# wavey-ai/soundkit

Measured on AMD Instinct MI355X. Metric: AAC-LC 1024-sample frames/s (whole node) + xrealtime, batch=4096 48 kHz stereo, higher is better.
Workload: dtype f32 (synthesis f32; s16 between the kernels as in the reference; FIR: the 16-bit samples as 2 x f16 exactly, the f32 taps as 2 x f16 to 2^-24, f32 accumulate; 1.0e-7 rel. RMS vs f64)

## Files before the change

soundkit_amd/csrc/fir_bf16.hip:

```cpp
#include "sk_device.h"

#include <cstdlib>
#include <type_traits>

namespace sk {

namespace {

typedef float f32x4 __attribute__((ext_vector_type(4)));
typedef __bf16 bf16x8 __attribute__((ext_vector_type(8)));
typedef uint32_t u32x4 __attribute__((ext_vector_type(4)));
typedef uint32_t u32x2 __attribute__((ext_vector_type(2)));

constexpr int kRing = 192;
constexpr int kPlaneBytes = 2 * kRing;
__host__ __device__ constexpr int row_bytes(int planes) { return planes * kPlaneBytes + 32; }
constexpr int kWindows = 10;
__device__ constexpr int kProducts[kWindows] = {1, 3, 6, 6, 6, 6, 6, 3, 3, 1};
__host__ __device__ constexpr int products_of(int s, bool in16) { return in16 && kProducts[s] > 5 ? 5 : kProducts[s]; }
__device__ constexpr int kProductsF16[kWindows] = {kFirProductsF16[0], kFirProductsF16[1], kFirProductsF16[2], kFirProductsF16[3], kFirProductsF16[4],
                                                     kFirProductsF16[5], kFirProductsF16[6], kFirProductsF16[7], kFirProductsF16[8], kFirProductsF16[9]};
__host__ __device__ constexpr int products_of(int s, bool in16, bool f16) { return f16 ? kProductsF16[s] : products_of(s, in16); }
#ifndef SK_BF_AHEAD
#define SK_BF_AHEAD 3
#endif
constexpr int kAhead = SK_BF_AHEAD;

__host__ __device__ constexpr int ring_index(int rho) { return ((rho % kRing) + kRing) % kRing; }

template <bool PACKED>
__device__ __forceinline__ size_t row_base_offset(const FirArgs &a, uint32_t row) {
    if (!PACKED) return (size_t)row * a.in_stride;
    const uint32_t sh = a.in_ch - 1;
    return (size_t)(row >> sh) * a.in_group_stride + (size_t)((row & sh) << 10);
}

template <bool PACKED>
__device__ __forceinline__ size_t time_offset(const FirArgs &a, uint32_t i) {
    return PACKED ? (size_t)(i >> 10) * a.in_block_stride + (size_t)(i & 1023) : (size_t)i;
}

__device__ __forceinline__ void split_pair(float x0, float x1, uint32_t &p1, uint32_t &p2, uint32_t &p3) {
    const uint32_t u0 = __float_as_uint(x0), u1 = __float_as_uint(x1);
    p1 = __builtin_amdgcn_perm(u1, u0, 0x07060302u);
    const float r0 = x0 - __uint_as_float(u0 & 0xffff0000u), r1 = x1 - __uint_as_float(u1 & 0xffff0000u);
    const uint32_t v0 = __float_as_uint(r0), v1 = __float_as_uint(r1);
    p2 = __builtin_amdgcn_perm(v1, v0, 0x07060302u);
    const float s0 = r0 - __uint_as_float(v0 & 0xffff0000u), s1 = r1 - __uint_as_float(v1 & 0xffff0000u);
    p3 = __builtin_amdgcn_perm(__float_as_uint(s1), __float_as_uint(s0), 0x07060302u);
}

__device__ __forceinline__ void split_pair16(uint32_t u, uint32_t &p1, uint32_t &p2) {
    const uint32_t m = u & 0xff00ff00u;
    const float a0 = (float)(int)(int16_t)(m & 0xffffu), a1 = (float)((int)m >> 16);
    const float b0 = (float)(u & 0xffu), b1 = (float)((u >> 16) & 0xffu);
    p1 = __builtin_amdgcn_perm(__float_as_uint(a1), __float_as_uint(a0), 0x07060302u);
    p2 = __builtin_amdgcn_perm(__float_as_uint(b1), __float_as_uint(b0), 0x07060302u);
}

__device__ __forceinline__ void split_pair16_f16(uint32_t u, uint32_t &p1, uint32_t &p2) { dev_split_pair16_f16(u, p1, p2); }

template <bool IN16>
struct Stage {
    using Elem = std::conditional_t<IN16, int16_t, float>;
    using Vec = std::conditional_t<IN16, u32x2, f32x4>;
    const Elem *base[4];
    uint32_t ok_mask;
    Vec v[2 * kAhead];
};

template <bool ALIGNED, bool PACKED, bool IN16>
__device__ __forceinline__ void stage_init(const FirArgs &a, int lane, uint32_t row0, Stage<IN16> &st) {
    st.ok_mask = 0;
    if (ALIGNED) {
#pragma unroll
        for (int ld = 0; ld < 4; ++ld) {
            const uint32_t r = row0 + 4 * ld + (lane >> 4);
            const bool ok = r < a.rows;
            const uint32_t phys = a.row_map ? a.row_map[ok ? r : 0] : (ok ? r : 0);
            if constexpr (IN16) st.base[ld] = a.in16 + row_base_offset<PACKED>(a, phys) + 4 * (lane & 15);
            else st.base[ld] = a.in + row_base_offset<PACKED>(a, phys) + 4 * (lane & 15);
            if (ok) st.ok_mask |= 1u << ld;
        }
    }
}

template <bool ALIGNED, bool PACKED, bool INTERIOR = false, bool IN16 = false>
__device__ __forceinline__ void stage_issue(const FirArgs &a, int lane, uint32_t row0, int64_t n, Stage<IN16> &st, int half, int slot) {
    using Vec = typename Stage<IN16>::Vec;
    using Elem = typename Stage<IN16>::Elem;
    if (ALIGNED) {
        const int64_t c0 = n - a.in_origin;
        const bool inside = c0 >= 0 && c0 + 64 <= (int64_t)a.in_frames;
        const bool one_block = !PACKED || (((uint32_t)c0 & 1023u) + 64u <= 1024u);
        if (INTERIOR || __builtin_expect(inside && one_block, 1)) {
            const size_t off = time_offset<PACKED>(a, (uint32_t)c0);
#pragma unroll
            for (int e2 = 0; e2 < 2; ++e2) {
                const int ld = 2 * half + e2, sl = 2 * slot + e2;
                st.v[sl] = *reinterpret_cast<const Vec *>(st.base[ld] + off);
            }
        } else {
            asm volatile("; chunk at an edge of the row" ::: "memory");
            const int64_t idx = c0 + 4 * (lane & 15);
            const bool in_range = (uint64_t)idx + 3 < (uint64_t)a.in_frames;
            const ptrdiff_t off = (ptrdiff_t)time_offset<PACKED>(a, (uint32_t)idx) - 4 * (lane & 15);
            const uint32_t sel = in_range ? st.ok_mask : 0u;
#pragma unroll
            for (int e2 = 0; e2 < 2; ++e2) {
                const int ld = 2 * half + e2, sl = 2 * slot + e2;
                const Elem *src = ((sel >> ld) & 1u) ? st.base[ld] + off : reinterpret_cast<const Elem *>(a.zeros) + 4 * lane;
                st.v[sl] = *reinterpret_cast<const Vec *>(src);
            }
        }
    } else if constexpr (!IN16) {
        const int64_t idx = n + lane - a.in_origin;
        const bool in_range = idx >= 0 && idx < (int64_t)a.in_frames;
        const size_t off = time_offset<PACKED>(a, (uint32_t)idx);
#pragma unroll
        for (int e2 = 0; e2 < 2; ++e2) {
            const int ld = 2 * half + e2, sl = 2 * slot + e2;
#pragma unroll
            for (int e = 0; e < 4; ++e) {
                const uint32_t r = row0 + 4 * ld + e;
                const bool ok = in_range && r < a.rows;
                const uint32_t phys = a.row_map ? a.row_map[r < a.rows ? r : 0] : r;
                st.v[sl][e] = ok ? a.in[row_base_offset<PACKED>(a, phys) + off] : 0.0f;
            }
        }
    }
}

template <bool ALIGNED, bool IN16, bool F16 = false>
__device__ __forceinline__ void stage_commit(unsigned char *lds, int lane, int ring_at, const Stage<IN16> &st, int half, int slot) {
#pragma unroll
    for (int e2 = 0; e2 < 2; ++e2) {
        const int ld = 2 * half + e2, sl = 2 * slot + e2;
        if constexpr (IN16) {
            uint32_t p1a, p2a, p1b, p2b;
            if constexpr (F16) {
                split_pair16_f16(st.v[sl][0], p1a, p2a);
                split_pair16_f16(st.v[sl][1], p1b, p2b);
            } else {
                split_pair16(st.v[sl][0], p1a, p2a);
                split_pair16(st.v[sl][1], p1b, p2b);
            }
            unsigned char *dst = lds + (4 * ld + (lane >> 4)) * row_bytes(2) + 2 * (ring_at + 4 * (lane & 15));
            *reinterpret_cast<u32x2 *>(dst) = (u32x2){p1a, p1b};
            *reinterpret_cast<u32x2 *>(dst + kPlaneBytes) = (u32x2){p2a, p2b};
        } else if (ALIGNED) {
            uint32_t p1a, p2a, p3a, p1b, p2b, p3b;
            split_pair(st.v[sl][0], st.v[sl][1], p1a, p2a, p3a);
            split_pair(st.v[sl][2], st.v[sl][3], p1b, p2b, p3b);
            unsigned char *dst = lds + (4 * ld + (lane >> 4)) * row_bytes(3) + 2 * (ring_at + 4 * (lane & 15));
            *reinterpret_cast<u32x2 *>(dst) = (u32x2){p1a, p1b};
            *reinterpret_cast<u32x2 *>(dst + kPlaneBytes) = (u32x2){p2a, p2b};
            *reinterpret_cast<u32x2 *>(dst + 2 * kPlaneBytes) = (u32x2){p3a, p3b};
        } else {
#pragma unroll
            for (int e = 0; e < 4; ++e) {
                uint32_t p1, p2, p3;
                split_pair(st.v[sl][e], 0.0f, p1, p2, p3);
                unsigned char *dst = lds + (4 * ld + e) * row_bytes(3) + 2 * (ring_at + lane);
                *reinterpret_cast<uint16_t *>(dst) = (uint16_t)p1;
                *reinterpret_cast<uint16_t *>(dst + kPlaneBytes) = (uint16_t)p2;
                *reinterpret_cast<uint16_t *>(dst + 2 * kPlaneBytes) = (uint16_t)p3;
            }
        }
    }
}

struct BFrag {
    u32x4 p[3];
};

__device__ __forceinline__ f32x4 mfma_bf16(const u32x4 &av, const u32x4 &bv, const f32x4 &c) {
    return dev_mfma_bf16(av, bv, c);
}

__device__ __forceinline__ f32x4 mfma_f16(const u32x4 &av, const u32x4 &bv, const f32x4 &c) { return dev_mfma_f16(av, bv, c); }

template <bool ALIGNED, bool PACKED, int OUT16, bool IN16 = false, bool F16 = false>
#ifndef SK_FIR_F16_WAVES
#define SK_FIR_F16_WAVES 3
#endif
__global__ __launch_bounds__(64, F16 ? SK_FIR_F16_WAVES : 2) void k_fir_48k_16k_bf16(FirArgs a, int32_t pair0, int32_t pair_end, int32_t pairs_per_seg,
                                                            uint32_t n_segs, int out_vec) {
    static_assert(!IN16 || ALIGNED, "s16 rows are read four samples at a time");
    static_assert(!F16 || IN16, "the f16 planes exist for s16 rows");
    constexpr int kPlanes = IN16 ? 2 : 3;
    __shared__ __attribute__((aligned(16))) unsigned char lds[16 * row_bytes(kPlanes)];

    const int lane = threadIdx.x;
    const int j = lane & 15, q = lane >> 4;
    const uint32_t group = blockIdx.x / n_segs, seg = blockIdx.x % n_segs;
    const uint32_t row0 = group * 16;
    const int32_t p_begin = pair0 + (int32_t)seg * pairs_per_seg;
    const int32_t p_end = p_begin + pairs_per_seg < pair_end ? p_begin + pairs_per_seg : pair_end;
    if (p_begin >= p_end) return;
    const int32_t p_last = p_end + 3;

    u32x4 af[kWindows][3];
    {
        const u32x4 *src = reinterpret_cast<const u32x4 *>(F16 ? a.afrag_f16 : a.afrag16);
        constexpr int kTapPlanes = F16 ? 2 : 3;
#pragma unroll
        for (int s = 0; s < kWindows; ++s)
#pragma unroll
            for (int k = 0; k < kTapPlanes; ++k) af[s][k] = src[(s * kTapPlanes + k) * 64 + lane];
    }

    Stage<IN16> st;
    stage_init<ALIGNED, PACKED, IN16>(a, lane, row0, st);

    const int64_t n_begin = (int64_t)96 * p_begin;
#pragma unroll
    for (int c = -2; c < 0; ++c) {
        stage_issue<ALIGNED, PACKED, false, IN16>(a, lane, row0, n_begin + 64 * c, st, 0, 0);
        stage_issue<ALIGNED, PACKED, false, IN16>(a, lane, row0, n_begin + 64 * c, st, 1, 1);
        stage_commit<ALIGNED, IN16, F16>(lds, lane, ring_index(64 * c), st, 0, 0);
        stage_commit<ALIGNED, IN16, F16>(lds, lane, ring_index(64 * c), st, 1, 1);
    }
#pragma unroll
    for (int i = 0; i < kAhead; ++i) stage_issue<ALIGNED, PACKED, false, IN16>(a, lane, row0, n_begin + 64 * (i >> 1), st, i & 1, i % kAhead);

    const uint32_t out_row = row0 + j;
    float *out_ptr = OUT16 ? nullptr
                           : a.out + (size_t)(out_row < a.rows ? out_row : 0) * a.out_stride +
                                 ((a.out_off && out_row < a.rows) ? a.out_off[out_row] : 0);

    const unsigned char *b_base = lds + j * row_bytes(kPlanes) + 16 * q;
    const unsigned char *b_base_wrap = b_base - (q >= 2 ? 2 * kRing : 0);
    auto read_b = [&](int rho) __attribute__((always_inline)) {
        BFrag f;
        const unsigned char *src = (ring_index(rho) + 32 > kRing ? b_base_wrap : b_base) + 2 * ring_index(rho);
#pragma unroll
        for (int p = 0; p < kPlanes; ++p) f.p[p] = *reinterpret_cast<const u32x4 *>(src + p * kPlaneBytes);
        return f;
    };

    const bool row_exists = out_row < a.rows;
    constexpr bool to_s16 = OUT16 != 0;
    float *out_lane = to_s16 ? nullptr : out_ptr + 4 * q;
    int16_t *out16_ptr = to_s16 ? a.out16 + (size_t)((row_exists ? out_row : 0) / (OUT16 ? OUT16 : 1)) * a.out16_stride * OUT16 : nullptr;
    auto store_tile = [&](auto itag, const f32x4 &vraw, int32_t pair, int parity) __attribute__((always_inline)) {
        const f32x4 v = F16 ? vraw * (1.0f / 2147483648.0f) : (IN16 ? vraw * (1.0f / 32768.0f) : vraw);
        constexpr bool INTERIOR = decltype(itag)::value;
        if (!INTERIOR && (pair < p_begin || pair >= p_end)) return;
        const int32_t rel_tile = 32 * pair + 16 * parity - (int32_t)a.out_first;
        const bool whole = INTERIOR || (out_vec && rel_tile >= 0 && rel_tile + 16 <= (int32_t)a.out_count);
        const bool row_ok = INTERIOR || row_exists;
        const int32_t rel = rel_tile + 4 * q;
        if (!to_s16) {
            if (INTERIOR || __builtin_expect(whole, 1)) {
                if (row_ok) *reinterpret_cast<f32x4 *>(out_lane + rel_tile) = v;
            } else {
                asm volatile("; tile at an edge of the output, or unaligned rows" ::: "memory");
#pragma unroll
                for (int r = 0; r < 4; ++r)
                    if (row_ok && rel + r >= 0 && rel + r < (int32_t)a.out_count) out_ptr[rel + r] = v[r];
            }
            return;
        }
        uint32_t mine01, mine23;
        if constexpr (IN16) {
            mine01 = dev_pack2_s16_scaled<F16 ? 31 : 15>(vraw[0], vraw[1]);
            mine23 = dev_pack2_s16_scaled<F16 ? 31 : 15>(vraw[2], vraw[3]);
        } else {
            mine01 = dev_pack2_s16(v[0], v[1]);
            mine23 = dev_pack2_s16(v[2], v[3]);
        }
        if (OUT16 == 2) {
            const uint32_t other01 = (uint32_t)__builtin_amdgcn_update_dpp(0, (int)mine01, 0xB1, 0xF, 0xF, true);
            const uint32_t other23 = (uint32_t)__builtin_amdgcn_update_dpp(0, (int)mine23, 0xB1, 0xF, 0xF, true);
            uint32_t w[4];
            w[0] = (mine01 & 0xffffu) | (other01 << 16);
            w[1] = (mine01 >> 16) | (other01 & 0xffff0000u);
            w[2] = (mine23 & 0xffffu) | (other23 << 16);
            w[3] = (mine23 >> 16) | (other23 & 0xffff0000u);
            if ((j & 1) == 0 && row_ok) {
                uint32_t *dst = reinterpret_cast<uint32_t *>(out16_ptr) + rel;
                if (INTERIOR || __builtin_expect(whole, 1)) {
                    *reinterpret_cast<u32x4 *>(dst) = (u32x4){w[0], w[1], w[2], w[3]};
                } else {
                    asm volatile("; tile at an edge of the output, or unaligned rows" ::: "memory");
#pragma unroll
                    for (int r = 0; r < 4; ++r)
                        if (rel + r >= 0 && rel + r < (int32_t)a.out_count) dst[r] = w[r];
                }
            }
        } else if (row_ok) {
            int16_t *dst = out16_ptr + rel;
            if (INTERIOR || __builtin_expect(whole, 1)) {
                *reinterpret_cast<u32x2 *>(dst) = (u32x2){mine01, mine23};
            } else {
                asm volatile("; tile at an edge of the output, or unaligned rows" ::: "memory");
#pragma unroll
                for (int r = 0; r < 4; ++r)
                    if (rel + r >= 0 && rel + r < (int32_t)a.out_count) dst[r] = (int16_t)((r < 2 ? mine01 : mine23) >> (16 * (r & 1)));
            }
        }
    };

    f32x4 acc[2][4];
#pragma unroll
    for (int par = 0; par < 2; ++par)
#pragma unroll
        for (int b = 0; b < 4; ++b) acc[par][b] = (f32x4){0.f, 0.f, 0.f, 0.f};

    BFrag bcur = read_b(-128);

    auto period = [&](auto ktag, auto itag, int32_t P, int64_t n_body) __attribute__((always_inline)) {
        constexpr int K = decltype(ktag)::value;
        constexpr bool INTERIOR = decltype(itag)::value;
#pragma unroll
        for (int wi = 0; wi < 3; ++wi) {
            const int step = 3 * K + wi;
            {
                __builtin_amdgcn_sched_barrier(0);
                stage_commit<ALIGNED, IN16, F16>(lds, lane, ring_index(64 * (step >> 1)), st, step & 1, step % kAhead);
                stage_issue<ALIGNED, PACKED, INTERIOR, IN16>(a, lane, row0, n_body + 64 * ((step + kAhead) >> 1), st,
                                                             (step + kAhead) & 1, step % kAhead);
            }
#pragma unroll
            for (int par = 0; par < 2; ++par) {
                const int t = 32 * step;
                const int rho_next = par == 0 ? t - 80 : t + 32 - 128;
                const BFrag bnext = read_b(rho_next);
#pragma unroll
                for (int prod = 0; prod < 6; ++prod) {
                    constexpr int hk[6] = {0, 1, 0, 1, 2, 0};
                    constexpr int xk[6] = {0, 0, 1, 1, 0, 2};
#pragma unroll
                    for (int d = 0; d < 4; ++d) {
                        const int s = 3 * d + wi;
                        if (s >= kWindows || prod >= products_of(s, IN16, F16)) continue;
                        f32x4 &c = acc[par][(K - d + 4) & 3];
                        const f32x4 c0 = (s == 0 && prod == 0) ? (f32x4){0.f, 0.f, 0.f, 0.f} : c;
                        if constexpr (F16) c = mfma_f16(af[s][hk[prod]], bcur.p[xk[prod]], c0);
                        else c = mfma_bf16(af[s][hk[prod]], bcur.p[xk[prod]], c0);
                    }
                }
                if (wi == 1 && par == 0) {
                    store_tile(itag, acc[0][(K + 1) & 3], P - 3, 0);
                    store_tile(itag, acc[1][(K + 1) & 3], P - 3, 1);
                }
                bcur = bnext;
            }
            if (INTERIOR) {
                int mfmas = 0;
#pragma unroll
                for (int d = 0; d < 4; ++d)
                    if (3 * d + wi < kWindows) mfmas += 2 * products_of(3 * d + wi, IN16, F16);
#pragma unroll
                for (int g = 0; g < mfmas; ++g) {
                    __builtin_amdgcn_sched_group_barrier(0x008, 1, 0);
                    __builtin_amdgcn_sched_group_barrier(0x002, 2, 0);
                }
            }
        }
    };

    using K0 = std::integral_constant<int, 0>;
    using K1 = std::integral_constant<int, 1>;
    using K2 = std::integral_constant<int, 2>;
    using K3 = std::integral_constant<int, 3>;
    const bool chunks_in_blocks = !PACKED || ((uint32_t)(n_begin - a.in_origin) & 63u) == 0;
    auto is_interior = [&](int32_t P0) {
        const int64_t n_body = (int64_t)96 * P0;
        const int64_t c_first = n_body + 64 * (kAhead >> 1) - a.in_origin, c_end = n_body + 64 * ((11 + kAhead) >> 1) + 64 - a.in_origin;
        const int64_t rel_first = (int64_t)32 * (P0 - 3) - (int64_t)a.out_first, rel_end = (int64_t)32 * P0 + 32 - (int64_t)a.out_first;
        return ALIGNED && chunks_in_blocks && c_first >= 0 && c_end <= (int64_t)a.in_frames && P0 - 3 >= p_begin && P0 < p_end &&
               out_vec && rel_first >= 0 && rel_end <= (int64_t)a.out_count && row0 + 16 <= a.rows;
    };
    auto general_body = [&](int32_t P0) __attribute__((always_inline)) {
        const int64_t n_body = (int64_t)96 * P0;
        if (P0 + 0 < p_last) period(K0{}, std::false_type{}, P0 + 0, n_body);
        if (P0 + 1 < p_last) period(K1{}, std::false_type{}, P0 + 1, n_body);
        if (P0 + 2 < p_last) period(K2{}, std::false_type{}, P0 + 2, n_body);
        if (P0 + 3 < p_last) period(K3{}, std::false_type{}, P0 + 3, n_body);
    };
    int32_t P0 = p_begin;
    for (; P0 < p_last && !is_interior(P0); P0 += 4) general_body(P0);
    for (; P0 < p_last && is_interior(P0); P0 += 4) {
        const int64_t n_body = (int64_t)96 * P0;
        period(K0{}, std::true_type{}, P0 + 0, n_body);
        period(K1{}, std::true_type{}, P0 + 1, n_body);
        period(K2{}, std::true_type{}, P0 + 2, n_body);
        period(K3{}, std::true_type{}, P0 + 3, n_body);
    }
    for (; P0 < p_last; P0 += 4) general_body(P0);
}

}

static bool fir_bf16_supported(const FirArgs &a) {
    const int64_t end_pair = ((int64_t)a.out_first + a.out_count + 31) / 32;
    return a.afrag16 != nullptr && end_pair <= 0x7ffffff0ll / 96 && a.out_count <= 0x7fffff00u;
}

hipError_t launch_fir_48k_16k(const FirArgs &a, hipStream_t s) {
    if (a.rows == 0 || a.out_count == 0) return hipSuccess;
    if (!fir_bf16_supported(a)) return hipErrorInvalidValue;
    const uint32_t groups = (a.rows + 15) / 16;
    const int64_t first_pair = ((int64_t)a.out_first / 32) & ~(int64_t)3;
    const int64_t end_pair = ((int64_t)a.out_first + a.out_count + 31) / 32;
    if (end_pair > 0x7ffffff0ll / 96 || a.out_count > 0x7fffff00u) return hipErrorInvalidValue;
    const uint32_t pairs = (uint32_t)(end_pair - first_pair);
    static const bool f16_rows = [] { const char *v = std::getenv("SK_FIR_S16_BF16"); return !(v && v[0] == '1'); }();
    const uint32_t waves_target = (a.in16 && a.afrag_f16 && f16_rows) ? 1024u * SK_FIR_F16_WAVES : 2048u;
    uint32_t n_segs = (waves_target + groups - 1) / groups;
    const uint32_t max_segs = pairs / 16 ? pairs / 16 : 1;
    if (n_segs > max_segs) n_segs = max_segs;
    uint32_t pps = (pairs + n_segs - 1) / n_segs;
    pps = (pps + 3) & ~3u;
    n_segs = (pairs + pps - 1) / pps;

    const bool strides_ok = a.in_block ? (a.in_block % 4 == 0 && a.in_block_stride % 4 == 0 && a.in_group_stride % 4 == 0)
                                       : (a.in_stride % 4 == 0);
    const bool aligned = ((a.in_origin & 3) == 0) && strides_ok && (a.in_frames % 4 == 0) &&
                         (a.in16 ? (((uintptr_t)a.in16 & 7) == 0) : (((uintptr_t)a.in & 15) == 0));
    if (a.out16 && (a.out16_ch < 1 || a.out16_ch > 2 || a.out_off || a.rows % a.out16_ch)) return hipErrorInvalidValue;
    const int out_vec = a.out16 ? ((a.out_first % 4 == 0) && (a.out16_stride * a.out16_ch) % 8 == 0 && (((uintptr_t)a.out16 & 15) == 0))
                                : ((a.out_first % 4 == 0) && (a.out_stride % 4 == 0) && (((uintptr_t)a.out & 15) == 0) &&
                                   a.out_off == nullptr);
    const bool packed = a.in_block != 0;
    if (packed && (a.in_block != 1024 || a.in_ch < 1 || a.in_ch > 2)) return hipErrorInvalidValue;
    const dim3 grid(groups * n_segs), block(64);
#define SK_FIR_LAUNCH(AL, PK, O16)                                                                                 \
    hipLaunchKernelGGL((k_fir_48k_16k_bf16<AL, PK, O16>), grid, block, 0, s, a, (int32_t)first_pair, (int32_t)end_pair, \
                       (int32_t)pps, n_segs, out_vec)
    if (a.in16) {
        if (!packed || !aligned) return hipErrorInvalidValue;
        const bool use_f16 = f16_rows;
#define SK_FIR_LAUNCH16(O16, F)                                                                                                    \
    hipLaunchKernelGGL((k_fir_48k_16k_bf16<true, true, O16, true, F>), grid, block, 0, s, a, (int32_t)first_pair, (int32_t)end_pair, \
                       (int32_t)pps, n_segs, out_vec)
        if (use_f16 && a.afrag_f16) {
            if (!a.out16) SK_FIR_LAUNCH16(0, true);
            else if (a.out16_ch == 2) SK_FIR_LAUNCH16(2, true);
            else SK_FIR_LAUNCH16(1, true);
        } else {
            if (!a.out16) SK_FIR_LAUNCH16(0, false);
            else if (a.out16_ch == 2) SK_FIR_LAUNCH16(2, false);
            else SK_FIR_LAUNCH16(1, false);
        }
#undef SK_FIR_LAUNCH16
    } else if (a.out16) {
        if (!packed) return hipErrorInvalidValue;
        if (aligned && a.out16_ch == 2) SK_FIR_LAUNCH(true, true, 2);
        else if (aligned) SK_FIR_LAUNCH(true, true, 1);
        else if (a.out16_ch == 2) SK_FIR_LAUNCH(false, true, 2);
        else SK_FIR_LAUNCH(false, true, 1);
    } else if (aligned && packed) SK_FIR_LAUNCH(true, true, 0);
    else if (aligned) SK_FIR_LAUNCH(true, false, 0);
    else if (packed) SK_FIR_LAUNCH(false, true, 0);
    else SK_FIR_LAUNCH(false, false, 0);
#undef SK_FIR_LAUNCH
    return hipGetLastError();
}

}
```

soundkit_amd/csrc/sk_device.h:

```cpp
#pragma once
#include <hip/hip_runtime.h>
#include <stdint.h>

#include "../../include/soundkit_amd.h"
#include "mp3_codebook_blob.h"

namespace sk {

struct SynthEntry {
    uint32_t off1024;
    uint32_t win;
};

struct SynthTask {
    uint32_t state;
    uint32_t begin;
    uint32_t count;
    uint32_t pad;
};

struct SynthTables {
    const float2 *tw_long;
    const float2 *tw_short;
    const float2 *w64;
    const float2 *w512;
    const float *win;
};

struct SynthArgs {
    const float *coeffs;
    float *pcm;
    int16_t *pcm16;
    float *delay;
    uint8_t *prev_shape;
    const SynthTask *tasks;
    const SynthEntry *entries;
    uint32_t n_tasks;
    uint32_t only_long;
    SynthTables t;
};

struct FrameSpan {
    uint32_t off1024;
    uint32_t channels;
};

hipError_t launch_aac_synth(const SynthArgs &a, hipStream_t s);
struct TailArgs {
    SynthArgs s;
    const uint32_t *afrag_f16;
    int16_t *out16;
    size_t out_stride;
    size_t stream_stride;
};
hipError_t launch_aac_tail(const TailArgs &ta, hipStream_t s);
hipError_t launch_aac_synth_pairs(const SynthArgs &a, bool with_short, hipStream_t s);
hipError_t launch_reset_streams(float *delay, uint8_t *shape, uint32_t *pns, const uint32_t *ids, uint32_t n, hipStream_t s);
hipError_t launch_zero_spans(float *base, const uint32_t *ids, uint32_t n, uint32_t span_floats, hipStream_t s);
hipError_t launch_frames_to_s16(const float *planar, int16_t *out, const FrameSpan *frames, uint32_t n, hipStream_t s);
hipError_t launch_dequantize(const int16_t *q, const int16_t *sf, float *out, size_t n, const float *pow43,
                             const float *sftab, hipStream_t s);

hipError_t launch_pcm_convert(int op, const void *in, void *out, size_t n, hipStream_t s);
hipError_t launch_interleave(const void *planar, void *out, size_t frames, uint32_t ch, int elem_bytes, hipStream_t s);
hipError_t launch_deinterleave(const void *in, void *planar, size_t frames, uint32_t ch, int elem_bytes, hipStream_t s);
hipError_t launch_deinterleave_s24(const uint8_t *in, int32_t *planar, size_t frames, uint32_t ch, hipStream_t s);
hipError_t launch_bytes_to_f32_planar(int variant, int fmt, const uint8_t *in, size_t frames, uint32_t ch, float *planar,
                                      hipStream_t s);
hipError_t launch_f32_planar_to_bytes(int fmt, const float *planar, size_t frames, uint32_t ch, uint8_t *out,
                                      hipStream_t s);
hipError_t launch_downmix_mono(const float *planar, size_t frames, uint32_t ch, float *mono, hipStream_t s);
hipError_t launch_exact_to_i16(int fmt, const uint8_t *in, size_t samples, uint8_t *out, hipStream_t s);
hipError_t launch_f32_planar_to_bytes_batch(int fmt, const float *planar, size_t batch, size_t plane_stride, size_t frames,
                                            uint32_t ch, uint8_t *out, hipStream_t s);

#ifdef __HIPCC__
__device__ __forceinline__ int dev_float_sample_to_i16(float x) {
    const float f = isfinite(x) ? fminf(fmaxf(x, -1.0f), 1.0f) : 0.0f;
    const double scaled = f < 0.0f ? (double)f * 32768.0 : (double)f * 32767.0;
    const int r = (int)round(scaled);
    return r < -32768 ? -32768 : (r > 32767 ? 32767 : r);
}

__device__ __forceinline__ int dev_float_sample_to_i16_f32(float x) {
    const float m = isfinite(x) ? fminf(fabsf(x), 1.0f) : 0.0f;
    const float a = m * 32768.0f;
    const float k = floorf(a);
    const float d = a - k;
    const int ki = (int)k;
    const int neg = ki + (d >= 0.5f ? 1 : 0);
    const int pos = ki + ((d - 0.5f >= m) ? 1 : 0) - ((d + 0.5f < m) ? 1 : 0);
    return x < 0.0f ? -neg : pos;
}
__device__ __forceinline__ int dev_float_sample_to_i16_v2(float x) {
    const float m = isfinite(x) ? fminf(fabsf(x), 1.0f) : 0.0f;
    const float a = m * 32768.0f;
    const float d = __builtin_amdgcn_fractf(a);
    const int ki = (int)a;
    const float mm = x < 0.0f ? 0.0f : m;
    const int r = ki + ((d - 0.5f >= mm) ? 1 : 0) - ((d + 0.5f < mm) ? 1 : 0);
    return x < 0.0f ? -r : r;
}
__device__ __forceinline__ int dev_float_sample_to_i16_presat(float x) {
    const float y = __builtin_fmaf(x, 0.0f, x);
    const double X = (double)y;
    const double half = __builtin_copysign(0.5, X);
    const double h = __builtin_fma(__builtin_fabs(X), -0.5, half);
    const double t = __builtin_fma(X, 32767.5, h);
    int k;
    asm("v_cvt_i32_f64 %0, %1" : "=v"(k) : "v"(t));
    return k;
}
__device__ __forceinline__ int dev_guarded_sample_to_i16_presat(float y) {
    const double X = (double)y;
    const double half = __builtin_copysign(0.5, X);
    const double h = __builtin_fma(__builtin_fabs(X), -0.5, half);
    const double t = __builtin_fma(X, 32767.5, h);
    int k;
    asm("v_cvt_i32_f64 %0, %1" : "=v"(k) : "v"(t));
    return k;
}
__device__ __forceinline__ uint32_t dev_pack2_s16(float lo, float hi) {
    typedef short s16x2_t __attribute__((ext_vector_type(2)));
    typedef float f32x2_t __attribute__((ext_vector_type(2)));
    const f32x2_t x = {lo, hi};
    const f32x2_t y = __builtin_elementwise_fma(x, (f32x2_t){0.0f, 0.0f}, x);
    const s16x2_t p = __builtin_amdgcn_cvt_pk_i16(dev_guarded_sample_to_i16_presat(y.x), dev_guarded_sample_to_i16_presat(y.y));
    return __builtin_bit_cast(uint32_t, p);
}

template <int EXP>
__device__ __forceinline__ int dev_scaled_sample_to_i16_presat(float acc) {
    constexpr double kScale = 1.0 / (double)(1ull << EXP);
    const double X = (double)acc;
    const double half = __builtin_copysign(0.5, X);
    const double h = __builtin_fma(__builtin_fabs(X), -0.5 * kScale, half);
    const double t = __builtin_fma(X, 32767.5 * kScale, h);
    int k;
    asm("v_cvt_i32_f64 %0, %1" : "=v"(k) : "v"(t));
    return k;
}
template <int EXP>
__device__ __forceinline__ uint32_t dev_pack2_s16_scaled(float lo, float hi) {
    typedef short s16x2_t __attribute__((ext_vector_type(2)));
    const s16x2_t p = __builtin_amdgcn_cvt_pk_i16(dev_scaled_sample_to_i16_presat<EXP>(lo), dev_scaled_sample_to_i16_presat<EXP>(hi));
    return __builtin_bit_cast(uint32_t, p);
}

typedef uint32_t sk_u32x4 __attribute__((ext_vector_type(4)));
typedef float sk_f32x4 __attribute__((ext_vector_type(4)));
__device__ __forceinline__ void dev_split_pair16_f16(uint32_t u, uint32_t &p1, uint32_t &p2) {
    typedef float f32x2 __attribute__((ext_vector_type(2)));
    const f32x2 f = {(float)(short)(u & 0xffffu), (float)((int)u >> 16)};
    const auto a = __builtin_amdgcn_cvt_pkrtz(f.x, f.y);
    const f32x2 r = f - (f32x2){(float)a[0], (float)a[1]};
    p1 = __builtin_bit_cast(uint32_t, a);
    p2 = __builtin_bit_cast(uint32_t, __builtin_amdgcn_cvt_pkrtz(r.x, r.y));
}
__device__ __forceinline__ sk_f32x4 dev_mfma_f16(const sk_u32x4 &av, const sk_u32x4 &bv, const sk_f32x4 &c) {
#if SK_MFMA_K16
    typedef _Float16 f16x4 __attribute__((ext_vector_type(4)));
    typedef uint32_t u32x2 __attribute__((ext_vector_type(2)));
    const sk_f32x4 t = __builtin_amdgcn_mfma_f32_16x16x16f16(__builtin_bit_cast(f16x4, (u32x2){av.x, av.y}), __builtin_bit_cast(f16x4, (u32x2){bv.x, bv.y}), c, 0, 0, 0);
    return __builtin_amdgcn_mfma_f32_16x16x16f16(__builtin_bit_cast(f16x4, (u32x2){av.z, av.w}), __builtin_bit_cast(f16x4, (u32x2){bv.z, bv.w}), t, 0, 0, 0);
#else
    typedef _Float16 f16x8 __attribute__((ext_vector_type(8)));
    return __builtin_amdgcn_mfma_f32_16x16x32_f16(__builtin_bit_cast(f16x8, av), __builtin_bit_cast(f16x8, bv), c, 0, 0, 0);
#endif
}
__device__ __forceinline__ sk_f32x4 dev_mfma_bf16(const sk_u32x4 &av, const sk_u32x4 &bv, const sk_f32x4 &c) {
#if SK_MFMA_K16
    typedef short s16x4 __attribute__((ext_vector_type(4)));
    typedef uint32_t u32x2 __attribute__((ext_vector_type(2)));
    const sk_f32x4 t = __builtin_amdgcn_mfma_f32_16x16x16bf16_1k(__builtin_bit_cast(s16x4, (u32x2){av.x, av.y}), __builtin_bit_cast(s16x4, (u32x2){bv.x, bv.y}), c, 0, 0, 0);
    return __builtin_amdgcn_mfma_f32_16x16x16bf16_1k(__builtin_bit_cast(s16x4, (u32x2){av.z, av.w}), __builtin_bit_cast(s16x4, (u32x2){bv.z, bv.w}), t, 0, 0, 0);
#else
    typedef __bf16 bf16x8 __attribute__((ext_vector_type(8)));
    return __builtin_amdgcn_mfma_f32_16x16x32_bf16(__builtin_bit_cast(bf16x8, av), __builtin_bit_cast(bf16x8, bv), c, 0, 0, 0);
#endif
}
__device__ constexpr int kFirProductsF16[10] = {1, 3, 3, 3, 3, 3, 3, 3, 1, 1};
#endif

struct FirArgs {
    const float *in;
    const int16_t *in16;
    float *out;
    int16_t *out16;
    size_t out16_stride;
    uint32_t out16_ch;
    const float *zeros;
    const uint32_t *afrag16;
    const uint32_t *afrag_f16;
    const float *taps;
    size_t in_stride, out_stride;
    uint32_t in_block, in_ch;
    size_t in_block_stride, in_group_stride;
    const uint32_t *row_map;
    const uint32_t *out_off;
    uint32_t rows;
    uint32_t in_frames;
    int32_t in_origin;
    uint32_t out_first;
    uint32_t out_count;
};
hipError_t launch_fir_48k_16k(const FirArgs &a, hipStream_t s);

struct SincArgs {
    const float *in;
    float *out;
    const float *sincs;
    const double *set_starts;
    const uint32_t *set_count;
    const uint32_t *row_set;
    uint32_t starts_stride;
    double step;
    const uint32_t *row_map;
    const uint32_t *out_off;
    size_t in_stride, out_stride;
    uint32_t rows, in_frames, out_count;
    int32_t in_origin;
    uint32_t n_sets;
    void *scratch;
    size_t scratch_bytes;
    int exact;
};
hipError_t launch_sinc_resample(const SincArgs &a, hipStream_t s);
uint32_t sinc_rows_per_block();
size_t sinc_mfma_scratch_bytes(uint32_t n_sets, uint32_t out_count, double step);

struct SincS16Args {
    const int16_t *in16;
    size_t stream_stride, frame_stride;
    uint32_t channels;
    uint32_t rows;
    uint32_t in_frames;
    int16_t *out16;
    float *out32;
    size_t out_stride;
    const float *sincs;
    const double *set_starts;
    const uint32_t *set_count;
    uint32_t starts_stride;
    double step;
    uint32_t out_count;
    void *scratch;
    size_t scratch_bytes;
};
hipError_t launch_sinc_rows_s16(const SincS16Args &a, hipStream_t s);

struct RowCopy {
    uint64_t src_off, dst_off;
    uint32_t count;
    uint32_t via_s16;
    uint32_t pieces = 1;
    uint32_t src_stride = 0;
};
hipError_t launch_row_copies(const float *src_base, float *dst_base, const RowCopy *jobs, uint32_t n_jobs, hipStream_t s);

constexpr uint32_t kMp3StateFloats = 1664;
struct Mp3Args {
    const float *xr;
    float *pcm;
    int16_t *pcm16;
    uint32_t planar_stride;
    float *state;
    const SynthTask *tasks;
    const SynthEntry *entries;
    uint32_t n_tasks;
    const float *imdct;
    const float *matrix;
    const float *window;
    const float *cs_ca;
};
hipError_t launch_mp3_hybrid(const Mp3Args &a, hipStream_t s);

struct Mp12Entry {
    uint32_t record;
    uint32_t pcm_off;
};
struct Mp12Args {
    const sk_mpa_frame_record *records;
    const uint32_t *bytes;
    float *pcm;
    int16_t *pcm16;
    uint32_t planar_stride;
    float *state;
    const SynthTask *tasks;
    const Mp12Entry *entries;
    uint32_t n_tasks;
    const float *matrix;
    const float *window;
    const float *scf;
};
hipError_t launch_mp12_synth(const Mp12Args &a, hipStream_t s);

constexpr uint32_t kMp3Rates = 9;
constexpr uint32_t kMp3BandRow = 40;
constexpr uint32_t kMp3Pow43 = 8208;
struct Mp3RequantRecord {
    uint32_t off;
    uint8_t slot, channels, flags, reserved;
    sk_mp3_requant_channel ch[2];
};
static_assert(sizeof(Mp3RequantRecord) % 4 == 0 && sizeof(Mp3RequantRecord) <= 256, "one word per lane");
struct Mp3RequantArgs {
    const Mp3RequantRecord *records;
    const int16_t *is;
    float *xr;
    uint32_t n;
    const float *pow43;
    const float *root4;
    const float *is_k;
    const uint16_t *bands;
    const uint8_t *pretab;
    const uint32_t *line_map;
};
hipError_t launch_mp3_requant(const Mp3RequantArgs &a, hipStream_t s);

static_assert(kMp3BlobRates == kMp3Rates, "one region table per band-table slot");
struct Mp3EntropyItem {
    uint32_t frame;
    uint32_t row;
    uint32_t record;
    uint8_t gr, ch, reserved[2];
};
struct Mp3EntropyCell {
    uint8_t scalefac_l[22];
    uint8_t scalefac_s[13][3];
    uint8_t preflag, intensity_scale, reserved;
    uint16_t part2_bits, nonzero_lines, part3_bits, reserved2;
    int32_t status;
};
static_assert(sizeof(Mp3EntropyCell) == 76, "packed by hand");
struct Mp3EntropyArgs {
    const uint32_t *blob;
    uint32_t lds_words;
    const sk_mp3_frame_item *frames;
    const uint8_t *bytes;
    const Mp3EntropyItem *items;
    uint32_t n_items;
    uint32_t lane_shift;
    int16_t *is;
    Mp3RequantRecord *records;
    Mp3EntropyCell *cells;
    int32_t *status;
};
hipError_t launch_mp3_entropy(const Mp3EntropyArgs &a, hipStream_t s);

}
#include "aac_entropy_core.h"
namespace sk {
constexpr int EC_SKIPPED = -199;
struct EntropyUnit {
    uint32_t word_offset;
    uint32_t byte_len;
    uint32_t off1024;
    uint32_t entry[2];
    uint32_t task;
};
struct EntropyTask {
    uint32_t stream, first, count;
    int32_t sf_index;
    uint32_t channels;
};
struct EntropyArgs {
    sk_ec::Tables t;
    const uint8_t *lds_blob;
    uint32_t lds_bytes;
    uint32_t lds_meta_off, lds_lut_off, lds_tuple_off, lds_sf_off, lds_swb_off, lds_pow_off;
    const uint32_t *words;
    const EntropyUnit *units;
    const EntropyTask *tasks;
    uint32_t n_tasks;
    uint32_t *pns_state;
    float *coeffs;
    SynthEntry *entries;
    int32_t *status;
    uint32_t n_units;
    sk_ec::Scratch *side;
    uint32_t *pns_start;
    uint32_t lane_shift;
    const uint32_t *order;
    const sk_ec::WireUnit *wire;
    const int16_t *quant;
};
hipError_t launch_aac_entropy_parallel(const EntropyArgs &a, hipStream_t s);

enum PackMode : uint8_t {
    kPackPlain = 0,
    kPackViaS16 = 1,
    kPackDirect = 2,
    kPackFromQ = 3,
    kPackPlainF32 = 4,
};
struct PackJob {
    const float *src0, *src1;
    uint8_t *dst;
    uint32_t frames;
    uint8_t ch_in, ch_out, bits, mode;
};
hipError_t launch_pack_jobs(const PackJob *jobs, uint32_t n_jobs, uint32_t max_frames, hipStream_t s);

constexpr uint32_t kPcmSliceSamples = 4096;
constexpr uint32_t kPcmCutFrames = 16;
struct PcmDirectJob {
    const uint8_t *src;
    uint8_t *dst;
    uint32_t frames;
    uint8_t fmt_in;
    uint8_t fmt_out;
    uint8_t ch_in, ch_out;
    uint32_t exact;
    uint32_t pad;
};
hipError_t launch_pcm_direct(const PcmDirectJob *jobs, uint32_t n_jobs, uint32_t max_samples , hipStream_t s);
struct PcmIngestJob {
    const uint8_t *src;
    float *dst0, *dst1;
    uint32_t frames;
    uint8_t fmt, ch, pad[2];
};
hipError_t launch_pcm_ingest(const PcmIngestJob *jobs, uint32_t n_jobs, uint32_t max_samples, hipStream_t s);

constexpr uint32_t kWideSliceFrames = 512;
constexpr uint8_t kWidePlanar = 0xff;
constexpr uint32_t kWideNoPeak = 0xffffffffu;
struct WideJob {
    const void *src;
    void *dst;
    uint64_t src_stride;
    uint64_t dst_stride;
    uint32_t frames;
    uint32_t peak;
    uint8_t fmt_in;
    uint8_t fmt_out;
    uint8_t ch_in, ch_out;
    uint32_t pad;
};
hipError_t launch_pcm_wide(const WideJob *jobs, uint32_t n_jobs, uint32_t n_peak_jobs, uint32_t max_frames, bool bytes_in, uint32_t *peaks,
                           hipStream_t s);
hipError_t launch_pcm_wide_one(const WideJob &job, uint32_t *peaks, hipStream_t s);
struct PcmWideIngestJob {
    const uint8_t *src;
    float *dst;
    uint64_t row_stride;
    uint32_t frames;
    uint8_t fmt, ch, pad[2];
};
hipError_t launch_pcm_wide_ingest(const PcmWideIngestJob *jobs, uint32_t n_jobs, uint32_t max_frames, hipStream_t s);

struct AiffElemJob {
    const uint8_t *src;
    uint8_t *dst;
    uint32_t samples;
    uint32_t enc;
};
hipError_t launch_aiff_elem(const AiffElemJob *jobs, uint32_t n_jobs, uint32_t max_samples, hipStream_t s);
struct AiffImaUnit {
    const uint8_t *src;
// ... 165 lines not shown
```

Before: 274.6 million.

## Use 32-bit buffer-resource addressing, early LDS reads, DPP stereo stores, mixed-FMA splits

Adds an A32 variant of the f16 s16-input FIR kernel that addresses input and output through buffer resources with 32-bit offsets, replacing 64-bit pointer arithmetic. It is selected when a host check confirms the extents fit in 2^31 bytes, and an env var can force the old path. The change also hoists the next B-fragment LDS reads ahead of the stage commit/issue, using a sched group barrier. Interior stereo s16 stores now let every lane write 8 bytes after one DPP exchange, instead of even lanes writing 16 bytes. The f16 residual split is rewritten with v_fma_mix instructions. Together these aim to cut VALU address work and instruction count in the hot loop, at the cost of more template variants and a risk of buffer out-of-range behaviour if the extents are computed wrongly.

```diff
diff --git a/soundkit_amd/csrc/fir_bf16.hip b/soundkit_amd/csrc/fir_bf16.hip
--- a/soundkit_amd/csrc/fir_bf16.hip
+++ b/soundkit_amd/csrc/fir_bf16.hip
@@ -25,6 +25,10 @@
 #define SK_BF_AHEAD 3
 #endif
 constexpr int kAhead = SK_BF_AHEAD;
+#ifndef SK_FIR_READ_EARLY
+#define SK_FIR_READ_EARLY 1
+#endif
+constexpr int kReadEarly = SK_FIR_READ_EARLY;
 
 __host__ __device__ constexpr int ring_index(int rho) { return ((rho % kRing) + kRing) % kRing; }
 
@@ -60,19 +64,36 @@
 
 __device__ __forceinline__ void split_pair16_f16(uint32_t u, uint32_t &p1, uint32_t &p2) { dev_split_pair16_f16(u, p1, p2); }
 
-template <bool IN16>
+typedef __amdgpu_buffer_rsrc_t rsrc_t;
+constexpr int kRsrcFlags = 0x00027000;
+
+template <bool IN16, bool A32 = false>
 struct Stage {
     using Elem = std::conditional_t<IN16, int16_t, float>;
     using Vec = std::conditional_t<IN16, u32x2, f32x4>;
-    const Elem *base[4];
+    std::conditional_t<A32, uint32_t, const Elem *> base[4];
+    rsrc_t rs;
     uint32_t ok_mask;
     Vec v[2 * kAhead];
 };
 
-template <bool ALIGNED, bool PACKED, bool IN16>
-__device__ __forceinline__ void stage_init(const FirArgs &a, int lane, uint32_t row0, Stage<IN16> &st) {
+template <bool ALIGNED, bool PACKED, bool IN16, bool A32>
+__device__ __forceinline__ void stage_init(const FirArgs &a, int lane, uint32_t row0, Stage<IN16, A32> &st) {
     st.ok_mask = 0;
-    if (ALIGNED) {
+    if constexpr (A32) {
+        static_assert(IN16 && ALIGNED && PACKED, "32-bit addressing is built for the frame-packed s16 rows");
+        const size_t g0 = row_base_offset<PACKED>(a, row0);
+        const uint32_t last = (a.rows - row0 < 16u ? a.rows - row0 : 16u) - 1u;
+        const size_t extent = row_base_offset<PACKED>(a, row0 + last) - g0 + time_offset<PACKED>(a, a.in_frames - 1u) + 1u;
+        st.rs = __builtin_amdgcn_make_buffer_rsrc(const_cast<int16_t *>(a.in16 + g0), 0, (int)(uint32_t)(2 * extent), kRsrcFlags);
+#pragma unroll
+        for (int ld = 0; ld < 4; ++ld) {
+            const uint32_t r = row0 + 4 * ld + (lane >> 4);
+            const bool ok = r < a.rows;
+            st.base[ld] = (uint32_t)(2 * (row_base_offset<PACKED>(a, ok ? r : row0) - g0)) + 8u * (lane & 15);
+            if (ok) st.ok_mask |= 1u << ld;
+        }
+    } else if (ALIGNED) {
 #pragma unroll
         for (int ld = 0; ld < 4; ++ld) {
             const uint32_t r = row0 + 4 * ld + (lane >> 4);
@@ -85,10 +106,10 @@
     }
 }
 
-template <bool ALIGNED, bool PACKED, bool INTERIOR = false, bool IN16 = false>
-__device__ __forceinline__ void stage_issue(const FirArgs &a, int lane, uint32_t row0, int64_t n, Stage<IN16> &st, int half, int slot) {
-    using Vec = typename Stage<IN16>::Vec;
-    using Elem = typename Stage<IN16>::Elem;
+template <bool ALIGNED, bool PACKED, bool INTERIOR = false, bool IN16 = false, bool A32 = false>
+__device__ __forceinline__ void stage_issue(const FirArgs &a, int lane, uint32_t row0, int64_t n, Stage<IN16, A32> &st, int half, int slot) {
+    using Vec = typename Stage<IN16, A32>::Vec;
+    using Elem = typename Stage<IN16, A32>::Elem;
     if (ALIGNED) {
         const int64_t c0 = n - a.in_origin;
         const bool inside = c0 >= 0 && c0 + 64 <= (int64_t)a.in_frames;
@@ -98,7 +119,8 @@
 #pragma unroll
             for (int e2 = 0; e2 < 2; ++e2) {
                 const int ld = 2 * half + e2, sl = 2 * slot + e2;
-                st.v[sl] = *reinterpret_cast<const Vec *>(st.base[ld] + off);
+                if constexpr (A32) st.v[sl] = __builtin_amdgcn_raw_buffer_load_b64(st.rs, st.base[ld], (int)(uint32_t)(2 * off), 0);
+                else st.v[sl] = *reinterpret_cast<const Vec *>(st.base[ld] + off);
             }
         } else {
             asm volatile("; chunk at an edge of the row" ::: "memory");
@@ -109,8 +131,14 @@
 #pragma unroll
             for (int e2 = 0; e2 < 2; ++e2) {
                 const int ld = 2 * half + e2, sl = 2 * slot + e2;
-                const Elem *src = ((sel >> ld) & 1u) ? st.base[ld] + off : reinterpret_cast<const Elem *>(a.zeros) + 4 * lane;
-                st.v[sl] = *reinterpret_cast<const Vec *>(src);
+                if constexpr (A32) {
+                    const bool use = ((sel >> ld) & 1u) != 0;
+                    const Vec got = __builtin_amdgcn_raw_buffer_load_b64(st.rs, st.base[ld] + (use ? (uint32_t)(2 * off) : 0u), 0, 0);
+                    st.v[sl] = use ? got : (Vec){0u, 0u};
+                } else {
+                    const Elem *src = ((sel >> ld) & 1u) ? st.base[ld] + off : reinterpret_cast<const Elem *>(a.zeros) + 4 * lane;
+                    st.v[sl] = *reinterpret_cast<const Vec *>(src);
+                }
             }
         }
     } else if constexpr (!IN16) {
@@ -131,8 +159,8 @@
     }
 }
 
-template <bool ALIGNED, bool IN16, bool F16 = false>
-__device__ __forceinline__ void stage_commit(unsigned char *lds, int lane, int ring_at, const Stage<IN16> &st, int half, int slot) {
+template <bool ALIGNED, bool IN16, bool F16 = false, bool A32 = false>
+__device__ __forceinline__ void stage_commit(unsigned char *lds, int lane, int ring_at, const Stage<IN16, A32> &st, int half, int slot) {
 #pragma unroll
     for (int e2 = 0; e2 < 2; ++e2) {
         const int ld = 2 * half + e2, sl = 2 * slot + e2;
@@ -180,7 +208,7 @@
 
 __device__ __forceinline__ f32x4 mfma_f16(const u32x4 &av, const u32x4 &bv, const f32x4 &c) { return dev_mfma_f16(av, bv, c); }
 
-template <bool ALIGNED, bool PACKED, int OUT16, bool IN16 = false, bool F16 = false>
+template <bool ALIGNED, bool PACKED, int OUT16, bool IN16 = false, bool F16 = false, bool A32 = false>
 #ifndef SK_FIR_F16_WAVES
 #define SK_FIR_F16_WAVES 3
 #endif
@@ -188,6 +216,7 @@
                                                             uint32_t n_segs, int out_vec) {
     static_assert(!IN16 || ALIGNED, "s16 rows are read four samples at a time");
     static_assert(!F16 || IN16, "the f16 planes exist for s16 rows");
+    static_assert(!A32 || F16, "32-bit addressing is built for the f16 form on s16 rows");
     constexpr int kPlanes = IN16 ? 2 : 3;
     __shared__ __attribute__((aligned(16))) unsigned char lds[16 * row_bytes(kPlanes)];
 
@@ -210,19 +239,19 @@
             for (int k = 0; k < kTapPlanes; ++k) af[s][k] = src[(s * kTapPlanes + k) * 64 + lane];
     }
 
-    Stage<IN16> st;
-    stage_init<ALIGNED, PACKED, IN16>(a, lane, row0, st);
+    Stage<IN16, A32> st;
+    stage_init<ALIGNED, PACKED, IN16, A32>(a, lane, row0, st);
 
     const int64_t n_begin = (int64_t)96 * p_begin;
 #pragma unroll
     for (int c = -2; c < 0; ++c) {
-        stage_issue<ALIGNED, PACKED, false, IN16>(a, lane, row0, n_begin + 64 * c, st, 0, 0);
-        stage_issue<ALIGNED, PACKED, false, IN16>(a, lane, row0, n_begin + 64 * c, st, 1, 1);
-        stage_commit<ALIGNED, IN16, F16>(lds, lane, ring_index(64 * c), st, 0, 0);
-        stage_commit<ALIGNED, IN16, F16>(lds, lane, ring_index(64 * c), st, 1, 1);
-    }
-#pragma unroll
-    for (int i = 0; i < kAhead; ++i) stage_issue<ALIGNED, PACKED, false, IN16>(a, lane, row0, n_begin + 64 * (i >> 1), st, i & 1, i % kAhead);
+        stage_issue<ALIGNED, PACKED, false, IN16, A32>(a, lane, row0, n_begin + 64 * c, st, 0, 0);
+        stage_issue<ALIGNED, PACKED, false, IN16, A32>(a, lane, row0, n_begin + 64 * c, st, 1, 1);
+        stage_commit<ALIGNED, IN16, F16, A32>(lds, lane, ring_index(64 * c), st, 0, 0);
+        stage_commit<ALIGNED, IN16, F16, A32>(lds, lane, ring_index(64 * c), st, 1, 1);
+    }
+#pragma unroll
+    for (int i = 0; i < kAhead; ++i) stage_issue<ALIGNED, PACKED, false, IN16, A32>(a, lane, row0, n_begin + 64 * (i >> 1), st, i & 1, i % kAhead);
 
     const uint32_t out_row = row0 + j;
     float *out_ptr = OUT16 ? nullptr
@@ -243,6 +272,27 @@
     constexpr bool to_s16 = OUT16 != 0;
     float *out_lane = to_s16 ? nullptr : out_ptr + 4 * q;
     int16_t *out16_ptr = to_s16 ? a.out16 + (size_t)((row_exists ? out_row : 0) / (OUT16 ? OUT16 : 1)) * a.out16_stride * OUT16 : nullptr;
+    const bool odd_lane = (j & 1) != 0;
+    const uint32_t sel_first = odd_lane ? 0x01000504u : 0x05040100u;
+    const uint32_t sel_second = odd_lane ? 0x03020706u : 0x07060302u;
+    rsrc_t out_rs;
+    uint32_t row_voff = 0, out_voff = 0;
+    if constexpr (A32) {
+        const uint32_t n_rows = a.rows - row0 < 16u ? a.rows - row0 : 16u;
+        if constexpr (to_s16) {
+            constexpr uint32_t kCh = OUT16 ? OUT16 : 1;
+            const uint32_t stream_bytes = (uint32_t)a.out16_stride * kCh * 2u;
+            out_rs = __builtin_amdgcn_make_buffer_rsrc(a.out16 + (size_t)(row0 / kCh) * a.out16_stride * kCh, 0,
+                                                       (int)((n_rows / kCh) * stream_bytes), kRsrcFlags);
+            row_voff = (j / kCh) * stream_bytes;
+            out_voff = row_voff + (kCh == 2 ? 16u * q + 8u * (j & 1) : 8u * q);
+        } else {
+            const uint32_t row_out_bytes = (uint32_t)a.out_stride * 4u;
+            out_rs = __builtin_amdgcn_make_buffer_rsrc(a.out + (size_t)row0 * a.out_stride, 0, (int)(n_rows * row_out_bytes), kRsrcFlags);
+            row_voff = j * row_out_bytes;
+            out_voff = row_voff + 16u * q;
+        }
+    }
     auto store_tile = [&](auto itag, const f32x4 &vraw, int32_t pair, int parity) __attribute__((always_inline)) {
         const f32x4 v = F16 ? vraw * (1.0f / 2147483648.0f) : (IN16 ? vraw * (1.0f / 32768.0f) : vraw);
         constexpr bool INTERIOR = decltype(itag)::value;
@@ -252,13 +302,20 @@
         const bool row_ok = INTERIOR || row_exists;
         const int32_t rel = rel_tile + 4 * q;
         if (!to_s16) {
-            if (INTERIOR || __builtin_expect(whole, 1)) {
-                if (row_ok) *reinterpret_cast<f32x4 *>(out_lane + rel_tile) = v;
+            if constexpr (INTERIOR && A32) {
+                __builtin_amdgcn_raw_buffer_store_b128(__builtin_bit_cast(u32x4, v), out_rs, out_voff, 4 * rel_tile, 0);
+            } else if (INTERIOR || __builtin_expect(whole, 1)) {
+                if constexpr (A32) {
+                    if (row_ok) __builtin_amdgcn_raw_buffer_store_b128(__builtin_bit_cast(u32x4, v), out_rs, out_voff, 4 * rel_tile, 0);
+                } else if (row_ok) *reinterpret_cast<f32x4 *>(out_lane + rel_tile) = v;
             } else {
                 asm volatile("; tile at an edge of the output, or unaligned rows" ::: "memory");
 #pragma unroll
                 for (int r = 0; r < 4; ++r)
-                    if (row_ok && rel + r >= 0 && rel + r < (int32_t)a.out_count) out_ptr[rel + r] = v[r];
+                    if (row_ok && rel + r >= 0 && rel + r < (int32_t)a.out_count) {
+                        if constexpr (A32) __builtin_amdgcn_raw_buffer_store_b32(__float_as_uint(v[r]), out_rs, row_voff + 4u * (uint32_t)(rel + r), 0, 0);
+                        else out_ptr[rel + r] = v[r];
+                    }
             }
             return;
         }
@@ -270,7 +327,13 @@
             mine01 = dev_pack2_s16(v[0], v[1]);
             mine23 = dev_pack2_s16(v[2], v[3]);
         }
-        if (OUT16 == 2) {
+        if constexpr (INTERIOR && OUT16 == 2) {
+            const uint32_t keep = odd_lane ? mine23 : mine01, send = odd_lane ? mine01 : mine23;
+            const uint32_t recv = (uint32_t)__builtin_amdgcn_update_dpp(0, (int)send, 0xB1, 0xF, 0xF, true);
+            const u32x2 w = {__builtin_amdgcn_perm(recv, keep, sel_first), __builtin_amdgcn_perm(recv, keep, sel_second)};
+            if constexpr (A32) __builtin_amdgcn_raw_buffer_store_b64(w, out_rs, out_voff, 4 * rel_tile, 0);
+            else *reinterpret_cast<u32x2 *>(reinterpret_cast<uint32_t *>(out16_ptr) + rel + 2 * (int)odd_lane) = w;
+        } else if (OUT16 == 2) {
             const uint32_t other01 = (uint32_t)__builtin_amdgcn_update_dpp(0, (int)mine01, 0xB1, 0xF, 0xF, true);
             const uint32_t other23 = (uint32_t)__builtin_amdgcn_update_dpp(0, (int)mine23, 0xB1, 0xF, 0xF, true);
             uint32_t w[4];
@@ -279,25 +342,34 @@
             w[2] = (mine23 & 0xffffu) | (other23 << 16);
             w[3] = (mine23 >> 16) | (other23 & 0xffff0000u);
             if ((j & 1) == 0 && row_ok) {
-                uint32_t *dst = reinterpret_cast<uint32_t *>(out16_ptr) + rel;
-                if (INTERIOR || __builtin_expect(whole, 1)) {
-                    *reinterpret_cast<u32x4 *>(dst) = (u32x4){w[0], w[1], w[2], w[3]};
+                uint32_t *dst = A32 ? nullptr : reinterpret_cast<uint32_t *>(out16_ptr) + rel;
+                if (__builtin_expect(whole, 1)) {
+                    if constexpr (A32) __builtin_amdgcn_raw_buffer_store_b128((u32x4){w[0], w[1], w[2], w[3]}, out_rs, row_voff + 16u * q, 4 * rel_tile, 0);
+                    else *reinterpret_cast<u32x4 *>(dst) = (u32x4){w[0], w[1], w[2], w[3]};
                 } else {
                     asm volatile("; tile at an edge of the output, or unaligned rows" ::: "memory");
 #pragma unroll
                     for (int r = 0; r < 4; ++r)
-                        if (rel + r >= 0 && rel + r < (int32_t)a.out_count) dst[r] = w[r];
+                        if (rel + r >= 0 && rel + r < (int32_t)a.out_count) {
+                            if constexpr (A32) __builtin_amdgcn_raw_buffer_store_b32(w[r], out_rs, row_voff + 4u * (uint32_t)(rel + r), 0, 0);
+                            else dst[r] = w[r];
+                        }
                 }
             }
         } else if (row_ok) {
-            int16_t *dst = out16_ptr + rel;
+            int16_t *dst = A32 ? nullptr : out16_ptr + rel;
             if (INTERIOR || __builtin_expect(whole, 1)) {
-                *reinterpret_cast<u32x2 *>(dst) = (u32x2){mine01, mine23};
+                if constexpr (A32) __builtin_amdgcn_raw_buffer_store_b64((u32x2){mine01, mine23}, out_rs, out_voff, 2 * rel_tile, 0);
+                else *reinterpret_cast<u32x2 *>(dst) = (u32x2){mine01, mine23};
             } else {
                 asm volatile("; tile at an edge of the output, or unaligned rows" ::: "memory");
 #pragma unroll
                 for (int r = 0; r < 4; ++r)
-                    if (rel + r >= 0 && rel + r < (int32_t)a.out_count) dst[r] = (int16_t)((r < 2 ? mine01 : mine23) >> (16 * (r & 1)));
+                    if (rel + r >= 0 && rel + r < (int32_t)a.out_count) {
+                        const int16_t one = (int16_t)((r < 2 ? mine01 : mine23) >> (16 * (r & 1)));
+                        if constexpr (A32) __builtin_amdgcn_raw_buffer_store_b16(one, out_rs, row_voff + 2u * (uint32_t)(rel + r), 0, 0);
+                        else dst[r] = one;
+                    }
             }
         }
     };
@@ -316,17 +388,20 @@
 #pragma unroll
         for (int wi = 0; wi < 3; ++wi) {
             const int step = 3 * K + wi;
+            BFrag bpar1, bstep;
             {
                 __builtin_amdgcn_sched_barrier(0);
-                stage_commit<ALIGNED, IN16, F16>(lds, lane, ring_index(64 * (step >> 1)), st, step & 1, step % kAhead);
-                stage_issue<ALIGNED, PACKED, INTERIOR, IN16>(a, lane, row0, n_body + 64 * ((step + kAhead) >> 1), st,
+                if (INTERIOR && kReadEarly >= 1) bpar1 = read_b(32 * step - 80);
+                if (INTERIOR && kReadEarly >= 2) bstep = read_b(32 * step + 32 - 128);
+                stage_commit<ALIGNED, IN16, F16, A32>(lds, lane, ring_index(64 * (step >> 1)), st, step & 1, step % kAhead);
+                stage_issue<ALIGNED, PACKED, INTERIOR, IN16, A32>(a, lane, row0, n_body + 64 * ((step + kAhead) >> 1), st,
                                                              (step + kAhead) & 1, step % kAhead);
             }
 #pragma unroll
             for (int par = 0; par < 2; ++par) {
                 const int t = 32 * step;
                 const int rho_next = par == 0 ? t - 80 : t + 32 - 128;
-                const BFrag bnext = read_b(rho_next);
+                const BFrag bnext = INTERIOR && kReadEarly > par ? (par == 0 ? bpar1 : bstep) : read_b(rho_next);
 #pragma unroll
                 for (int prod = 0; prod < 6; ++prod) {
                     constexpr int hk[6] = {0, 1, 0, 1, 2, 0};
@@ -352,6 +427,7 @@
 #pragma unroll
                 for (int d = 0; d < 4; ++d)
                     if (3 * d + wi < kWindows) mfmas += 2 * products_of(3 * d + wi, IN16, F16);
+                if (kReadEarly) __builtin_amdgcn_sched_group_barrier(0x100, kPlanes * kReadEarly, 0);
 #pragma unroll
                 for (int g = 0; g < mfmas; ++g) {
                     __builtin_amdgcn_sched_group_barrier(0x008, 1, 0);
@@ -399,6 +475,17 @@
     return a.afrag16 != nullptr && end_pair <= 0x7ffffff0ll / 96 && a.out_count <= 0x7fffff00u;
 }
 
+static bool fir_addr32_fits(const FirArgs &a) {
+    static const bool forced64 = [] { const char *v = std::getenv("SK_FIR_ADDR64"); return v && v[0] == '1'; }();
+    if (forced64 || a.row_map || a.out_off || a.in_block != 1024 || a.in_ch < 1 || a.in_ch > 2) return false;
+    constexpr uint64_t kLimit = 1ull << 31;
+    if (a.in_group_stride >= kLimit || a.in_block_stride >= kLimit || a.out16_stride >= kLimit || a.out_stride >= kLimit) return false;
+    const uint64_t in_bytes = 2 * ((uint64_t)(16 / a.in_ch) * a.in_group_stride + 2048 + ((uint64_t)a.in_frames / 1024 + 1) * a.in_block_stride + 1024);
+    const uint64_t out_bytes = a.out16 ? 2 * (16 * (uint64_t)a.out16_stride + 2 * (uint64_t)a.out_count + 64)
+                                       : 4 * (16 * (uint64_t)a.out_stride + (uint64_t)a.out_count + 64);
+    return in_bytes < kLimit && out_bytes < kLimit;
+}
+
 hipError_t launch_fir_48k_16k(const FirArgs &a, hipStream_t s) {
     if (a.rows == 0 || a.out_count == 0) return hipSuccess;
     if (!fir_bf16_supported(a)) return hipErrorInvalidValue;
@@ -433,10 +520,14 @@
     if (a.in16) {
         if (!packed || !aligned) return hipErrorInvalidValue;
         const bool use_f16 = f16_rows;
-#define SK_FIR_LAUNCH16(O16, F)                                                                                                    \
-    hipLaunchKernelGGL((k_fir_48k_16k_bf16<true, true, O16, true, F>), grid, block, 0, s, a, (int32_t)first_pair, (int32_t)end_pair, \
+#define SK_FIR_LAUNCH16(O16, F, ...)                                                                                               \
+    hipLaunchKernelGGL((k_fir_48k_16k_bf16<true, true, O16, true, F, ##__VA_ARGS__>), grid, block, 0, s, a, (int32_t)first_pair, (int32_t)end_pair, \
                        (int32_t)pps, n_segs, out_vec)
-        if (use_f16 && a.afrag_f16) {
+        if (use_f16 && a.afrag_f16 && fir_addr32_fits(a)) {
+            if (!a.out16) SK_FIR_LAUNCH16(0, true, true);
+            else if (a.out16_ch == 2) SK_FIR_LAUNCH16(2, true, true);
+            else SK_FIR_LAUNCH16(1, true, true);
+        } else if (use_f16 && a.afrag_f16) {
             if (!a.out16) SK_FIR_LAUNCH16(0, true);
             else if (a.out16_ch == 2) SK_FIR_LAUNCH16(2, true);
             else SK_FIR_LAUNCH16(1, true);
diff --git a/soundkit_amd/csrc/sk_device.h b/soundkit_amd/csrc/sk_device.h
--- a/soundkit_amd/csrc/sk_device.h
+++ b/soundkit_amd/csrc/sk_device.h
@@ -149,13 +149,21 @@
 
 typedef uint32_t sk_u32x4 __attribute__((ext_vector_type(4)));
 typedef float sk_f32x4 __attribute__((ext_vector_type(4)));
+#ifndef SK_SPLIT_MIX
+#define SK_SPLIT_MIX 1
+#endif
 __device__ __forceinline__ void dev_split_pair16_f16(uint32_t u, uint32_t &p1, uint32_t &p2) {
     typedef float f32x2 __attribute__((ext_vector_type(2)));
     const f32x2 f = {(float)(short)(u & 0xffffu), (float)((int)u >> 16)};
     const auto a = __builtin_amdgcn_cvt_pkrtz(f.x, f.y);
+    p1 = __builtin_bit_cast(uint32_t, a);
+#if SK_SPLIT_MIX
+    asm("v_fma_mixlo_f16 %0, %1, -1.0, %2 op_sel_hi:[1,0,0]" : "=v"(p2) : "v"(p1), "v"(f.x));
+    asm("v_fma_mixhi_f16 %0, %1, -1.0, %2 op_sel:[1,0,0] op_sel_hi:[1,0,0]" : "+v"(p2) : "v"(p1), "v"(f.y));
+#else
     const f32x2 r = f - (f32x2){(float)a[0], (float)a[1]};
-    p1 = __builtin_bit_cast(uint32_t, a);
     p2 = __builtin_bit_cast(uint32_t, __builtin_amdgcn_cvt_pkrtz(r.x, r.y));
+#endif
 }
 __device__ __forceinline__ sk_f32x4 dev_mfma_f16(const sk_u32x4 &av, const sk_u32x4 &bv, const sk_f32x4 &c) {
 #if SK_MFMA_K16
```

New measurement: 277.9 million (median of 6 runs). +1.2%, better.
